# ohinder/OnePhase.jl

Hardware: AMD Instinct MI355X
Metric: KKT factor+solve/sec (fp64) at n+m~1e5, nnz~2e6 (higher is better)
Workload: dtype f64

## Files before the change

include/okkt.h:

```cpp
#ifndef OKKT_H
#define OKKT_H

#include <stdint.h>

#ifdef __cplusplus
extern "C" {
#endif

typedef struct okkt_solver_s* okkt_handle;
typedef struct okkt_kkt_s* okkt_kkt_handle;

typedef enum {
  OKKT_OK = 0,
  OKKT_ERR_INVALID = -1,
  OKKT_ERR_NO_DEVICE = -2,
  OKKT_ERR_HIP = -3,
  OKKT_ERR_ALLOC = -4,
  OKKT_ERR_INTERNAL = -5
} okkt_status;

#define OKKT_SYM_DEFINITE 0
#define OKKT_SYM_SYMMETRIC 1

#define OKKT_KKT_SCHUR 0
// ... 122 lines not shown
int okkt_get_schur_dev(okkt_handle h, double* d_S, int64_t ld);
int okkt_schur_condense(okkt_handle h, const double* rhs, double* r2, int64_t nrhs);
int okkt_schur_condense_dev(okkt_handle h, const double* d_rhs, double* d_r2, int64_t nrhs);
int okkt_schur_expand(okkt_handle h, const double* rhs, const double* x2, double* x, int64_t nrhs);
int okkt_schur_expand_dev(okkt_handle h, const double* d_rhs, const double* d_x2, double* d_x, int64_t nrhs);
int okkt_schur_factor(okkt_handle h, const double* S_or_NULL, int64_t ld, okkt_inertia* inertia_S, okkt_inertia* inertia_total);
int okkt_schur_factor_dev(okkt_handle h, const double* d_S_or_NULL, int64_t ld, okkt_inertia* inertia_S, okkt_inertia* inertia_total);
int okkt_schur_dense_solve(okkt_handle h, const double* r2, double* x2, int64_t nrhs);
int okkt_schur_dense_solve_dev(okkt_handle h, const double* d_r2, double* d_x2, int64_t nrhs);
int okkt_schur_solve(okkt_handle h, const double* rhs, double* sol, int64_t nrhs);
int okkt_schur_solve_dev(okkt_handle h, const double* d_rhs, double* d_sol, int64_t nrhs);
int okkt_schur_get_factor(okkt_handle h, double* LD, int64_t ld, int32_t* ipiv);
typedef struct {
  double seconds_device;
  int64_t arena_bytes;
  int64_t nonfinite;
  int32_t status;
  double flops;
} okkt_selinv_info;
int okkt_selinv(okkt_handle h, okkt_selinv_info* info );
int okkt_get_inverse_diag(okkt_handle h, double* d_out);
int okkt_get_inverse_diag_dev(okkt_handle h, double* d_out);
int okkt_get_inverse_on_pattern(okkt_handle h, double* zval, int64_t* nnz);
int okkt_get_inverse_on_pattern_dev(okkt_handle h, double* d_zval);
int okkt_get_inverse_csc(okkt_handle h, int64_t* colptr, int64_t* rowval, double* val, int64_t* nnz);
int okkt_logdet(okkt_handle h, double* logabsdet, int32_t* sign);

#define OKKT_SCALE_NONE 0
#define OKKT_SCALE_RUIZ 1
#define OKKT_SCALE_USER 2
typedef struct {
  int32_t mode, sweeps;
  double rowmax_min, rowmax_max;
  int64_t zero_rows;
} okkt_scaling_info;
int okkt_set_scaling(okkt_handle h, int mode, int32_t sweeps ,
                     const double* s_user );
int okkt_get_scaling(okkt_handle h, double* s_out , okkt_scaling_info* info );
int okkt_get_scaling_dev(okkt_handle h, double* d_s_out);

int okkt_get_diag(okkt_handle h, double* d_out );
int okkt_get_factor_csc(okkt_handle h, int64_t* colptr_out, int64_t* rowval_out, double* val_out, int64_t* nnz_out);

int okkt_dev_alloc(okkt_handle h, int64_t bytes, void** d_ptr_out);
int okkt_dev_free(okkt_handle h, void* d_ptr);
int okkt_dev_upload(okkt_handle h, void* d_dst, const void* src, int64_t bytes);
int okkt_dev_download(okkt_handle h, void* dst, const void* d_src, int64_t bytes);
int okkt_set_early_exit(okkt_handle h, int enable);
void* okkt_get_stream(okkt_handle h);
int okkt_profile_dominant(okkt_handle h, int enable);
int okkt_get_profile(okkt_handle h, int64_t* n_launches, double* total_ms, double* total_flops);
int64_t okkt_debug_dataflow_queue(int32_t nfronts, const int32_t* f, const int32_t* k, int32_t workers, int32_t group,
                                  int32_t* tasks, int64_t cap, double* model_us);


int okkt_dist_set_partition(okkt_handle h, int nparts, int part_id);
int okkt_dist_info(okkt_handle h, int64_t* cb_doubles, int64_t* cv_doubles, int64_t* n_boundary,
                   double* part_flops_out , double* top_flops_out);
int okkt_dist_get_owner(okkt_handle h, int64_t* sn_owner_out, int64_t* col_owner_out, int64_t* sn_parent_out);
int okkt_dist_factor_local(okkt_handle h, const double* d_nzval, int64_t n, int64_t m, int sym_kind);
int okkt_dist_cb(okkt_handle h, double* d_buf, int unpack);
int okkt_dist_factor_top(okkt_handle h);
int okkt_dist_counts(okkt_handle h, int64_t out[4]);
int okkt_dist_finish(okkt_handle h, const int64_t total[4]);
int okkt_dist_solve_begin(okkt_handle h, const double* d_rhs);
int okkt_dist_cv(okkt_handle h, double* d_buf, int unpack);
int okkt_dist_solve_top(okkt_handle h);
int okkt_dist_x(okkt_handle h, double* d_buf, int mode);
int okkt_dist_solve_end(okkt_handle h);

int okkt_dist_unique_id(void* id_out );
int okkt_dist_comm_init(okkt_handle h, int nranks, int rank, const void* id );
int okkt_dist_comm_destroy(okkt_handle h);
int okkt_dist_factor(okkt_handle h, const double* d_nzval, int64_t n, int64_t m, int sym_kind, okkt_inertia* inertia_out);
int okkt_dist_solve(okkt_handle h, const double* d_rhs, double* d_sol);

typedef struct {
  double delta_start, delta_min, delta_max, delta_inc, delta_dec, delta_zero;
  int32_t ItRefine_Num;
  int32_t max_it;
} okkt_kkt_pars;

typedef struct {
  double assemble_ms;
  double upload_ms;
  double shift_ms;
  double factor_ms;
  double rhs_ms;
  double solve_ms;
  double refine_ms;
  double kkt_err_ms;
  double direction_ms;
  int32_t n_solves;
  int32_t reserved;
} okkt_kkt_timers;

typedef struct {
  double error_D, error_P, error_mu, overall, rhs_norm, ratio;
} okkt_kkt_error;

int okkt_kkt_default_pars(okkt_kkt_pars* pars);
int okkt_kkt_create(okkt_kkt_handle* out, const okkt_opts* opts, int kkt_kind);
int okkt_kkt_destroy(okkt_kkt_handle k);
const char* okkt_kkt_last_error(okkt_kkt_handle k);
okkt_handle okkt_kkt_linear_solver(okkt_kkt_handle k);
int okkt_kkt_set_structure(okkt_kkt_handle k, int64_t n, int64_t m,
// ... 55 lines not shown
```

onephase.jl_amd/_lib.py:

```python
import ctypes as C
import os

import numpy as np

_HERE = os.path.dirname(os.path.abspath(__file__))
LIB_PATH = os.environ.get("OKKT_LIB_PATH", os.path.join(_HERE, "libonephase_kkt.so"))

OKKT_SYM_DEFINITE = 0
OKKT_SYM_SYMMETRIC = 1
OKKT_KKT_SCHUR = 0
OKKT_KKT_SYMMETRIC = 1
OKKT_KKT_CLEVER_SYMMETRIC = 2
OKKT_KKT_SCHUR_DIRECT = 3
OKKT_RESCALE = {"none": 0, "u_only": 1, "u_and_x": 2}
OKKT_SCALE_NONE = 0
OKKT_SCALE_RUIZ = 1
OKKT_SCALE_USER = 2
OKKT_SCALE = {"none": OKKT_SCALE_NONE, "ruiz": OKKT_SCALE_RUIZ, "user": OKKT_SCALE_USER}

OKKT_OK = 0
OKKT_ERR_INVALID = -1
OKKT_ERR_NO_DEVICE = -2
OKKT_ERR_HIP = -3
OKKT_ERR_ALLOC = -4
# ... 187 lines not shown
    "okkt_get_etree": (C.c_int, [_vp, _i64p, _i64p]),
    "okkt_factor": (C.c_int, [_vp, _f64p, C.c_int64, C.c_int64, C.c_int, C.POINTER(OkktInertia)]),
    "okkt_factor_dev": (C.c_int, [_vp, _vp, C.c_int64, C.c_int64, C.c_int, C.POINTER(OkktInertia)]),
    "okkt_solve": (C.c_int, [_vp, _f64p, _f64p, C.c_int64]),
    "okkt_solve_dev": (C.c_int, [_vp, _vp, _vp, C.c_int64]),
    "okkt_residual": (C.c_int, [_vp, _f64p, _f64p, _f64p, _f64p, C.c_int64, _f64p]),
    "okkt_residual_dev": (C.c_int, [_vp, _vp, _vp, _vp, _vp, C.c_int64, _f64p]),
    "okkt_solve_refine": (C.c_int, [_vp, _f64p, _f64p, _f64p, C.c_int64, C.c_int32, C.c_double, C.POINTER(OkktRefineInfo), _f64p]),
    "okkt_solve_refine_dev": (C.c_int, [_vp, _vp, _vp, _vp, C.c_int64, C.c_int32, C.c_double, C.POINTER(OkktRefineInfo), _f64p]),
    "okkt_solve_gmres": (C.c_int, [_vp, _f64p, _f64p, _f64p, C.c_int64, C.c_int32, C.c_int32, C.c_double, C.POINTER(OkktGmresInfo),
                                   _f64p]),
    "okkt_solve_gmres_dev": (C.c_int, [_vp, _vp, _vp, _vp, C.c_int64, C.c_int32, C.c_int32, C.c_double, C.POINTER(OkktGmresInfo), _f64p]),
    "okkt_condest": (C.c_int, [_vp, _f64p, C.c_int32, C.POINTER(OkktCondestInfo)]),
    "okkt_condest_dev": (C.c_int, [_vp, _vp, C.c_int32, C.POINTER(OkktCondestInfo)]),
    "okkt_condest_indices": (C.c_int64, [_vp, _i64p, C.c_int64]),
    "okkt_forward_error": (C.c_int, [_vp, _f64p, _f64p, _f64p, C.c_int64, _f64p, _f64p]),
    "okkt_forward_error_dev": (C.c_int, [_vp, _vp, _vp, _vp, C.c_int64, _f64p, _f64p]),
    "okkt_set_schur": (C.c_int, [_vp, C.c_int64, _i64p]),
    "okkt_factor_schur": (C.c_int, [_vp, _f64p, C.c_int64, C.c_int64, C.c_int, C.POINTER(OkktInertia)]),
    "okkt_factor_schur_dev": (C.c_int, [_vp, _vp, C.c_int64, C.c_int64, C.c_int, C.POINTER(OkktInertia)]),
    "okkt_get_schur": (C.c_int, [_vp, _f64p, C.c_int64]),
    "okkt_get_schur_dev": (C.c_int, [_vp, _vp, C.c_int64]),
    "okkt_schur_condense": (C.c_int, [_vp, _f64p, _f64p, C.c_int64]),
    "okkt_schur_condense_dev": (C.c_int, [_vp, _vp, _vp, C.c_int64]),
    "okkt_schur_expand": (C.c_int, [_vp, _f64p, _f64p, _f64p, C.c_int64]),
    "okkt_schur_expand_dev": (C.c_int, [_vp, _vp, _vp, _vp, C.c_int64]),
    "okkt_schur_factor": (C.c_int, [_vp, _f64p, C.c_int64, C.POINTER(OkktInertia), C.POINTER(OkktInertia)]),
    "okkt_schur_factor_dev": (C.c_int, [_vp, _vp, C.c_int64, C.POINTER(OkktInertia), C.POINTER(OkktInertia)]),
    "okkt_schur_dense_solve": (C.c_int, [_vp, _f64p, _f64p, C.c_int64]),
    "okkt_schur_dense_solve_dev": (C.c_int, [_vp, _vp, _vp, C.c_int64]),
    "okkt_schur_solve": (C.c_int, [_vp, _f64p, _f64p, C.c_int64]),
    "okkt_schur_solve_dev": (C.c_int, [_vp, _vp, _vp, C.c_int64]),
    "okkt_schur_get_factor": (C.c_int, [_vp, _f64p, C.c_int64, C.POINTER(C.c_int32)]),
    "okkt_selinv": (C.c_int, [_vp, C.POINTER(OkktSelinvInfo)]),
    "okkt_get_inverse_diag": (C.c_int, [_vp, _f64p]),
    "okkt_get_inverse_diag_dev": (C.c_int, [_vp, _vp]),
    "okkt_get_inverse_on_pattern": (C.c_int, [_vp, _f64p, _i64p]),
    "okkt_get_inverse_on_pattern_dev": (C.c_int, [_vp, _vp]),
    "okkt_get_inverse_csc": (C.c_int, [_vp, _i64p, _i64p, _f64p, _i64p]),
    "okkt_logdet": (C.c_int, [_vp, _f64p, C.POINTER(C.c_int32)]),
    "okkt_set_scaling": (C.c_int, [_vp, C.c_int, C.c_int32, _f64p]),
    "okkt_get_scaling": (C.c_int, [_vp, _f64p, C.POINTER(OkktScalingInfo)]),
    "okkt_get_scaling_dev": (C.c_int, [_vp, _vp]),
    "okkt_get_diag": (C.c_int, [_vp, _f64p]),
    "okkt_get_factor_csc": (C.c_int, [_vp, _i64p, _i64p, _f64p, _i64p]),
    "okkt_dev_alloc": (C.c_int, [_vp, C.c_int64, C.POINTER(_vp)]),
    "okkt_dev_free": (C.c_int, [_vp, _vp]),
    "okkt_dev_upload": (C.c_int, [_vp, _vp, _vp, C.c_int64]),
    "okkt_dev_download": (C.c_int, [_vp, _vp, _vp, C.c_int64]),
    "okkt_get_stream": (_vp, [_vp]),
    "okkt_profile_dominant": (C.c_int, [_vp, C.c_int]),
    "okkt_get_profile": (C.c_int, [_vp, _i64p, _f64p, _f64p]),
    "okkt_debug_dataflow_queue": (C.c_int64, [C.c_int32, C.POINTER(C.c_int32), C.POINTER(C.c_int32), C.c_int32, C.c_int32, C.POINTER(C.c_int32), C.c_int64, _f64p]),
    "okkt_dist_set_partition": (C.c_int, [_vp, C.c_int, C.c_int]),
    "okkt_dist_info": (C.c_int, [_vp, _i64p, _i64p, _i64p, _f64p, _f64p]),
    "okkt_dist_get_owner": (C.c_int, [_vp, _i64p, _i64p, _i64p]),
    "okkt_dist_factor_local": (C.c_int, [_vp, _vp, C.c_int64, C.c_int64, C.c_int]),
    "okkt_dist_cb": (C.c_int, [_vp, _vp, C.c_int]),
    "okkt_dist_factor_top": (C.c_int, [_vp]),
    "okkt_dist_counts": (C.c_int, [_vp, _i64p]),
    "okkt_dist_finish": (C.c_int, [_vp, _i64p]),
    "okkt_dist_solve_begin": (C.c_int, [_vp, _vp]),
    "okkt_dist_cv": (C.c_int, [_vp, _vp, C.c_int]),
    "okkt_dist_solve_top": (C.c_int, [_vp]),
    "okkt_dist_x": (C.c_int, [_vp, _vp, C.c_int]),
    "okkt_dist_solve_end": (C.c_int, [_vp]),
    "okkt_dist_unique_id": (C.c_int, [_vp]),
    "okkt_dist_comm_init": (C.c_int, [_vp, C.c_int, C.c_int, _vp]),
    "okkt_dist_comm_destroy": (C.c_int, [_vp]),
    "okkt_dist_factor": (C.c_int, [_vp, _vp, C.c_int64, C.c_int64, C.c_int, C.POINTER(OkktInertia)]),
    "okkt_dist_solve": (C.c_int, [_vp, _vp, _vp]),
    "okkt_kkt_default_pars": (C.c_int, [C.POINTER(OkktKktPars)]),
    "okkt_kkt_create": (C.c_int, [C.POINTER(_vp), C.POINTER(OkktOpts), C.c_int]),
    "okkt_kkt_destroy": (C.c_int, [_vp]),
    "okkt_kkt_last_error": (C.c_char_p, [_vp]),
    "okkt_kkt_linear_solver": (_vp, [_vp]),
    "okkt_kkt_set_structure": (C.c_int, [_vp, C.c_int64, C.c_int64, _i64p, _i64p, _i64p, _i64p, C.c_int]),
    "okkt_kkt_form_system": (C.c_int, [_vp, _f64p, _f64p, _f64p, _f64p]),
    "okkt_kkt_diag_min": (C.c_int, [_vp, _f64p]),
    "okkt_kkt_factor": (C.c_int, [_vp, C.c_double, C.POINTER(OkktInertia)]),
    "okkt_kkt_factor_trial": (C.c_int, [_vp, C.c_double, C.POINTER(OkktInertia)]),
    "okkt_kkt_get_timers": (C.c_int, [_vp, C.POINTER(OkktKktTimers)]),
    "okkt_kkt_get_direction": (C.c_int, [_vp, _f64p, _f64p, _f64p]),
    "okkt_kkt_ipopt_strategy": (C.c_int, [_vp, C.c_double, C.POINTER(OkktKktPars), C.POINTER(C.c_int32), _f64p]),
    "okkt_kkt_compute_directions": (C.c_int, [_vp, C.c_int32, _f64p, C.c_int32, _f64p, _f64p, _f64p, C.POINTER(OkktKktError)]),
    "okkt_kkt_is_diag_dom": (C.c_int, [_vp, C.POINTER(C.c_int32)]),
    "okkt_kkt_diag_dom_warnings": (C.c_int, [_vp, C.POINTER(C.c_int32)]),
    "okkt_kkt_estimate_y_tilde": (C.c_int, [_vp, _f64p, _f64p]),
    "okkt_kkt_system_rhs": (C.c_int, [_vp, _f64p, _f64p, _f64p, _f64p, _f64p, C.c_double, C.c_double, C.c_double, C.c_double, C.c_double, _f64p, _f64p, _f64p]),
    "okkt_kkt_compute_direction": (C.c_int, [_vp, _f64p, _f64p, _f64p, C.c_int32, _f64p, _f64p, _f64p, C.POINTER(OkktKktError)]),
    "okkt_kkt_get_matrix": (C.c_int, [_vp, _i64p, _i64p, _i64p, _i64p, _f64p]),
    "okkt_kkt_get_schur_diag": (C.c_int, [_vp, _f64p]),
    "okkt_kkt_get_dense_rows": (C.c_int, [_vp, _i64p, _i64p]),
    "okkt_kkt_set_ls_refine": (C.c_int, [_vp, C.c_int32, C.c_double]),
    "okkt_kkt_set_ls_scaling": (C.c_int, [_vp, C.c_int, C.c_int32]),
    "okkt_kkt_condest": (C.c_int, [_vp, C.c_int32, C.POINTER(OkktCondestInfo)]),
    "okkt_kkt_direction_error_bound": (C.c_int, [_vp, _f64p]),
    "okkt_kkt_compute_indicies": (C.c_int, [_vp, _f64p, C.POINTER(C.c_int64)]),
    "okkt_kkt_get_indicies": (C.c_int, [_vp, _i64p, _i64p, _i64p, _f64p, _f64p, _f64p, _f64p]),
    "okkt_kkt_get_clever_vectors": (C.c_int, [_vp, _f64p, _f64p, _f64p, _f64p, _f64p]),
    "okkt_kkt_set_rescale": (C.c_int, [_vp, C.c_int, C.c_double, C.c_double]),
    "okkt_kkt_set_direction": (C.c_int, [_vp, _f64p, _f64p, _f64p]),
    "okkt_kkt_max_step_primal": (C.c_int, [_vp, _f64p, C.c_double, _f64p, _f64p]),
    "okkt_kkt_s_bound_ok": (C.c_int, [_vp, _f64p, _f64p, C.c_double, C.POINTER(C.c_int32)]),
    "okkt_kkt_dual_step_range": (C.c_int, [_vp, _f64p, _f64p, C.c_double, C.c_double, _f64p, _f64p, _f64p]),
    "okkt_kkt_predicted_reduction": (C.c_int, [_vp, _f64p, C.c_double, C.c_double, C.c_double, C.c_double, _f64p]),
# ... 44 lines not shown
```

onephase.jl_amd/csrc/dataflow.hip:

```cpp
#include "front_device.h"

#include <algorithm>
#include <type_traits>
#include <cstdio>
#include <cstdlib>

namespace okkt {

#define OKKT_HIP_TRY(expr)                                                         \
  do {                                                                             \
    hipError_t e__ = (expr);                                                       \
    if (e__ != hipSuccess)                                                         \
      return std::string(#expr) + ": " + hipGetErrorString(e__);                   \
  } while (0)

typedef double d2_t __attribute__((ext_vector_type(2)));
constexpr int kDfThreadsC = 512;
#ifndef OKKT_DF_STAGES
#define OKKT_DF_STAGES 2
#endif
#ifndef OKKT_DF_KC
#define OKKT_DF_KC 32
#endif
#ifndef OKKT_DF_STAGGER
#define OKKT_DF_STAGGER 1
#endif
constexpr bool kDfStagger = OKKT_DF_STAGGER != 0;
#ifndef OKKT_DF_PROG
#define OKKT_DF_PROG 0
#endif
constexpr bool kDfProg = OKKT_DF_PROG != 0;
#ifndef OKKT_DF_MACRO
#define OKKT_DF_MACRO 0
#endif
#ifndef OKKT_DF_ROT
#define OKKT_DF_ROT 0
#endif
#ifndef OKKT_DF_CHAIN_BUILD
#define OKKT_DF_CHAIN_BUILD 0
#endif
constexpr bool kDfChain = OKKT_DF_CHAIN_BUILD != 0;
#ifndef OKKT_DF_LOG_BUILD
#define OKKT_DF_LOG_BUILD 0
#endif
constexpr bool kDfLog = OKKT_DF_LOG_BUILD != 0;
#ifndef OKKT_DF_PIPE
#define OKKT_DF_PIPE 0
#endif
#ifndef OKKT_DF_MULTI
#define OKKT_DF_MULTI 1
#endif
constexpr bool kDfMulti = OKKT_DF_MULTI != 0;
constexpr bool kDfPipe = OKKT_DF_PIPE != 0;
constexpr bool kDfRot = OKKT_DF_ROT != 0;
constexpr bool kDfMacro = OKKT_DF_MACRO != 0;
constexpr int kDfDiagMfmaWaves = 6;
constexpr int kDfKC = OKKT_DF_KC;
constexpr int kDfStages = OKKT_DF_STAGES;

__device__ __forceinline__ void st_sc1_f64x2(double* p, d2_t v) { asm volatile("global_store_dwordx4 %0, %1, off sc1" : : "v"(p), "v"(v) : "memory"); }
__device__ __forceinline__ int ld_state(const int* p) { return __hip_atomic_load(p, __ATOMIC_RELAXED, __HIP_MEMORY_SCOPE_AGENT); }

__device__ __forceinline__ int df_block_lo(int b, int KB, int k, int f) { return b < KB ? b * 128 : min(k + (b - KB) * 128, f); }

__device__ __forceinline__ void df_trsm_tile(const DevPlan& P, int s, int q, int r0, int rlim, double* sm) {
  constexpr int NBLK = 4, NB = 128, NPAIR = NBLK * (NBLK + 1) / 2;
  int tid_ = threadIdx.x;
  asm volatile("" : "+v"(tid_));
  const int tid = tid_, lane = tid & 63, wv = tid >> 6;
  const int col0 = P.sn_col0[s];
  const int k = P.sn_col0[s + 1] - col0;
  const int f = (int)(P.row_ptr[s + 1] - P.row_ptr[s]);
  const int j0 = q * NB;
  const int nb = min(NB, k - j0);
  double* F = P.arena + P.front_pos[s];
  double* Wb = P.wbuf + P.wbuf_pos[s] + (size_t)j0 * f;
  const double* X = P.invl + P.invl_pos[s] + (size_t)q * NB * NB;
  double* rdv = sm + NPAIR * kIB * kIB;
  const int row = r0 + wv * 16 + (lane & 15);
  const int rowc = min(row, f - 1);
  const bool valid = row < rlim;
  const int lk = lane >> 4, li = lane & 3;
  double t[NBLK * 8];
#pragma unroll
  for (int qq = 0; qq < NBLK * 8; ++qq) {
    const int c = 4 * qq + lk;
    t[qq] = keep_f64(F[(size_t)(j0 + min(c, nb - 1)) * f + rowc], c < nb && valid);
  }
  {
    const int e = tid * 2;
    const int cc = e / kIB, rr = e - cc * kIB;
#pragma unroll
    for (int bi = 0; bi < NBLK; ++bi)
#pragma unroll
      for (int bp = 0; bp <= bi; ++bp) {
        double v[2];
        const int gr = bi * kIB + rr, gc = bp * kIB + cc;
#pragma unroll
        for (int u = 0; u < 2; ++u) {
          const double* src = bp == bi ? X + (gr + u) + (size_t)gc * NB
                                       : F + (size_t)(j0 + min(gc, nb - 1)) * f + j0 + min(gr + u, nb - 1);
          v[u] = keep_f64(*src, gr + u < nb && gc < nb);
        }
        double* dst = sm + (bi * (bi + 1) / 2 + bp) * kIB * kIB + e;
        dst[0] = v[0]; dst[1] = v[1];
      }
    if (tid < NB) rdv[tid] = tid < nb ? 1.0 / P.dvals[col0 + j0 + tid] : 0.0;
// ... 712 lines not shown
#pragma unroll
      for (int cg = 0; cg < 4; ++cg) {
        const int c = r0 + 16 * (ucode[u] >> 2) + cg * 4 + l4;
        if (c >= rlim) continue;
        double* colp = F + (size_t)c * f;
        if (r + 1 < rlim && r >= c) {
          st_sc1_f64x2(colp + r, (d2_t){acc[u][cg][0], acc[u][cg][1]});
        } else {
          if (r < rlim && r >= c) st_agent_f64(colp + r, acc[u][cg][0]);
          if (r + 1 < rlim && r + 1 >= c) st_agent_f64(colp + r + 1, acc[u][cg][1]);
        }
      }
    }
    asm volatile("s_waitcnt vmcnt(0)" ::: "memory");
    __syncthreads();
    if (wave == 0) __hip_atomic_store(diag_state, dval, __ATOMIC_RELAXED, __HIP_MEMORY_SCOPE_AGENT);
  } else {
    asm volatile("s_waitcnt lgkmcnt(0)" ::: "memory");
    __syncthreads();
    double* Tl = sm;
#pragma unroll
    for (int u = 0; u < NU; ++u) {
      if (!unit_on(u)) continue;
      const int r = 32 * (ucode[u] & 3) + 2 * l15;
#pragma unroll
      for (int cg = 0; cg < 4; ++cg) {
        const int c = 16 * (ucode[u] >> 2) + cg * 4 + l4;
        const d2_t v = (d2_t){acc[u][cg][0], acc[u][cg][1]};
        __builtin_memcpy(Tl + (size_t)c * kDfTileLd + r, &v, 16);
      }
    }
    asm volatile("s_waitcnt vmcnt(0)" ::: "memory");
    __syncthreads();
    if (wave == 0) __hip_atomic_store(row_state, dval, __ATOMIC_RELAXED, __HIP_MEMORY_SCOPE_AGENT);
  }
  return true;
}

template <int CTRL>
__device__ __forceinline__ double df_row_ror(double v) {
  const int lo = __builtin_amdgcn_update_dpp(0, __double2loint(v), CTRL, 0xf, 0xf, false);
  const int hi = __builtin_amdgcn_update_dpp(0, __double2hiint(v), CTRL, 0xf, 0xf, false);
  return __hiloint2double(hi, lo);
}

template <int KC, int STAGES, bool MULTI, bool STAGGER>
__device__ __forceinline__ void df_syrk_tiles(const DevPlan& P, int s, int j0, int nb, int i, int R_, int j, int KB, int k, double* sm, long long* marks, int* pub0 = nullptr, int pub_stride = 0, int pub_val = 0) {
  constexpr int NW = kSyrkNW;
  constexpr int kDfKC = KC;
  const int R = MULTI ? R_ : 1;
  constexpr int DMA = 2 * (kDfKC / NW);
  constexpr int WCW = 128 / (NW / 2);
  constexpr int NCG = WCW / 4;
  int tid_ = threadIdx.x;
  asm volatile("" : "+v"(tid_));
  const int tid = tid_, lane = tid & 63, wv = tid >> 6;
  const int f = (int)(P.row_ptr[s + 1] - P.row_ptr[s]);
  const int ct0 = df_block_lo(j, KB, k, f), clim = df_block_lo(j + 1, KB, k, f);
  const int cbase = ct0 + (wv >> 1) * WCW;
  double* F = P.arena + P.front_pos[s];
  double* Fc = F + (j >= KB ? P.cb_shift[s] : 0);
  const double* Wcol = P.wbuf + P.wbuf_pos[s] + (size_t)j0 * f + lane * 2;
  const double* Lg = F + (size_t)j0 * f + ct0 + lane * 2;
  const int l15 = lane & 15, l4 = lane >> 4;
  const int quad = (lane >> 2) & 3;
  int grp1 = quad, grp2 = quad, grp3 = quad;
  if constexpr (kDfRot) {
    grp1 = __builtin_amdgcn_update_dpp(0, quad, 0x124, 0xf, 0xf, false);
    grp2 = __builtin_amdgcn_update_dpp(0, quad, 0x128, 0xf, 0xf, false);
    grp3 = __builtin_amdgcn_update_dpp(0, quad, 0x12C, 0xf, 0xf, false);
  }
  auto col_of = [&](int cg) {
    if constexpr (!kDfRot) return cbase + cg * 4 + l4;
    const int m = cg & 3;
    return cbase + (cg >> 2) * 16 + (m == 0 ? quad : m == 1 ? grp1 : m == 2 ? grp2 : grp3) * 4 + l4;
  };
  const int nchunk = (nb + kDfKC - 1) / kDfKC;
  const int total = R * nchunk;
  auto issue = [&](int g) {
    const int r = g / nchunk, ch = g - r * nchunk;
    const double* Wg = Wcol + df_block_lo(i + r, KB, k, f);
    double* slot = sm + (size_t)(g % STAGES) * 2 * kDfKC * kSyrkLd;
#pragma unroll
    for (int qq = 0; qq < kDfKC / NW; ++qq) {
      const int prow = qq * NW + wv;
      const int p = ch * kDfKC + prow;
      const double* wsrc = p < nb ? Wg + (size_t)p * f : P.zero_page + lane * 2;
      const double* lsrc = p < nb ? Lg + (size_t)p * f : P.zero_page + lane * 2;
      __builtin_amdgcn_global_load_lds(wsrc, (lds_void_t*)(slot + prow * kSyrkLd), 16, 0, 0);
      __builtin_amdgcn_global_load_lds(lsrc, (lds_void_t*)(slot + (kDfKC + prow) * kSyrkLd), 16, 0, 0);
    }
  };
  d2_t raw[NCG][2];
  auto load_c = [&](int r) {
    const int rbase = df_block_lo(i + r, KB, k, f) + (wv & 1) * 64;
#pragma unroll
    for (int cg = 0; cg < NCG; ++cg) {
      const int c = col_of(cg);
      const double* colp = Fc + (size_t)min(c, clim - 1) * f;
#pragma unroll
      for (int h = 0; h < 2; ++h) {
        const int rr = rbase + 2 * l15 + 32 * h;
        __builtin_memcpy(&raw[cg][h], colp + min(rr, f - 2), 16);
      }
    }
  };
  double acc[NCG][4];
  auto mask_c = [&](int r) {
    const int rbase = df_block_lo(i + r, KB, k, f) + (wv & 1) * 64;
    const int rlim = df_block_lo(i + r + 1, KB, k, f);
#pragma unroll
    for (int cg = 0; cg < NCG; ++cg) {
      const int c = col_of(cg);
#pragma unroll
      for (int h = 0; h < 2; ++h) {
        const int rr = rbase + 2 * l15 + 32 * h;
        const int shift = rr - min(rr, f - 2);
        const double e0 = shift == 0 ? raw[cg][h][0] : raw[cg][h][1];
        acc[cg][2 * h] = keep_f64(e0, rr < rlim && c < clim && rr >= c);
        acc[cg][2 * h + 1] = keep_f64(raw[cg][h][1], shift == 0 && rr + 1 < rlim && c < clim && rr + 1 >= c);
      }
    }
  };
  load_c(0);
  asm volatile("" ::: "memory");
  mask_c(0);
#pragma unroll
  for (int g = 0; g < STAGES - 1; ++g) if (g < total) issue(g);
  int pend_r = -1;
  int plain_until = 0;
  const int pre = min(2, nchunk - 1);
  int r = 0, ch = 0;
  for (int g = 0; g < total; ++g) {
    {
      const int later = g < plain_until ? 0 : min(STAGES - 2, total - 1 - g);
      if (later >= 2) asm volatile("s_waitcnt vmcnt(%0)" ::"n"(2 * DMA) : "memory");
      else if (later == 1) asm volatile("s_waitcnt vmcnt(%0)" ::"n"(DMA) : "memory");
      else asm volatile("s_waitcnt vmcnt(0)" ::: "memory");
    }
    __builtin_amdgcn_s_barrier();
    if constexpr (MULTI) {
      if (pend_r >= 0) {
        if (tid == 0) __hip_atomic_store(pub0 + (size_t)pend_r * pub_stride, pub_val, __ATOMIC_RELAXED, __HIP_MEMORY_SCOPE_AGENT);
        pend_r = -1;
      }
    }
    if (marks && g == 0 && tid == 0) { marks[0] = wall_clock64(); marks[3] = -(long long)clock64(); }
    const bool late = STAGGER && wv >= 4;
    const bool more = g + STAGES - 1 < total;
    if (more && !late) issue(g + STAGES - 1);
    if constexpr (MULTI) { if (ch == pre && r + 1 < R) { load_c(r + 1); plain_until = g + STAGES; } }
    const int rt0 = df_block_lo(i + r, KB, k, f), rlim = df_block_lo(i + r + 1, KB, k, f);
    const int rbase = rt0 + (wv & 1) * 64;
    const bool active = !(rbase + 63 < cbase) && rbase < rlim && cbase < clim && !(kDfChain && P.df_dbg_half && nb >= 256 && (g & 1));
    if (active) {
      const double* slot = sm + (size_t)(g % STAGES) * 2 * kDfKC * kSyrkLd;
      const double* bw = slot + (wv & 1) * 64 + 2 * l15;
      const double* bl = slot + kDfKC * kSyrkLd + (wv >> 1) * WCW + (kDfRot ? l15 : (lane & 3));
      if constexpr (kDfRot || !kDfPipe) {
  #pragma unroll
        for (int kk = 0; kk < kDfKC / 4; ++kk) {
          if (kk == (KC / 8) && more && late) issue(g + STAGES - 1);
          double bv[4];
  #pragma unroll
          for (int rb = 0; rb < 4; ++rb) bv[rb] = bw[(kk * 4 + l4) * kSyrkLd + (rb & 1) + 32 * (rb >> 1)];
  #pragma unroll
          for (int half = 0; half < NCG / 4; ++half) {
            double av[4];
  #pragma unroll
            for (int qq = 0; qq < 4; ++qq) if (!kDfRot || qq == 0) av[qq] = bl[(kk * 4 + l4) * kSyrkLd + (half * 4 + qq) * 4];
            if constexpr (kDfRot) {
              av[1] = df_row_ror<0x124>(av[0]);
              av[2] = df_row_ror<0x128>(av[0]);
              av[3] = df_row_ror<0x12C>(av[0]);
            }
  #pragma unroll
            for (int qq = 0; qq < 4; ++qq)
  #pragma unroll
              for (int rb = 0; rb < 4; ++rb)
                acc[half * 4 + qq][rb] = __builtin_amdgcn_mfma_f64_4x4x4f64(av[qq], bv[rb], acc[half * 4 + qq][rb], 0, 0, 1 );
          }
        }
      } else {
        static_assert(NCG == 8, "two halves of four column groups per k-step");
        const unsigned ba = (unsigned)(size_t)(bl + l4 * kSyrkLd);
        const unsigned bb = (unsigned)(size_t)(bw + l4 * kSyrkLd);
        d2_t B0[2], B1[2], A0[2], A1[2];
        auto ldb = [&](int kk, d2_t (&bq)[2]) {
          const unsigned ad = bb + kk * 4 * kSyrkLd * 8;
          asm volatile("ds_read_b128 %0, %2\n\tds_read_b128 %1, %2 offset:256" : "=&v"(bq[0]), "=&v"(bq[1]) : "v"(ad));
        };
        auto lda = [&](int kk, int half, d2_t (&aq)[2]) {
          const unsigned ad = ba + kk * 4 * kSyrkLd * 8 + half * 128;
          asm volatile("ds_read2_b64 %0, %2 offset1:4\n\tds_read2_b64 %1, %2 offset0:8 offset1:12" : "=&v"(aq[0]), "=&v"(aq[1]) : "v"(ad));
        };
        ldb(0, B0);
        lda(0, 0, A0);
#pragma unroll
        for (int st = 0; st < 2 * (kDfKC / 4); ++st) {
          const int kk = st >> 1, half = st & 1;
          d2_t (&Ac)[2] = (st & 1) ? A1 : A0;
          d2_t (&Bc)[2] = (kk & 1) ? B1 : B0;
          if (st == 2 * (KC / 8) && more && late) issue(g + STAGES - 1);
          if (st + 1 < 2 * (kDfKC / 4)) {
            const int k2 = (st + 1) >> 1, h2 = (st + 1) & 1;
            if (h2 == 0) ldb(k2, (k2 & 1) ? B1 : B0);
            lda(k2, h2, ((st + 1) & 1) ? A1 : A0);
          }
          if (st + 1 >= 2 * (kDfKC / 4)) asm volatile("s_waitcnt lgkmcnt(0)" : "+v"(Ac[0]), "+v"(Ac[1]), "+v"(Bc[0]), "+v"(Bc[1]));
          else if (((st + 1) & 1) == 0) asm volatile("s_waitcnt lgkmcnt(4)" : "+v"(Ac[0]), "+v"(Ac[1]), "+v"(Bc[0]), "+v"(Bc[1]));
          else asm volatile("s_waitcnt lgkmcnt(2)" : "+v"(Ac[0]), "+v"(Ac[1]), "+v"(Bc[0]), "+v"(Bc[1]));
#pragma unroll
          for (int qq = 0; qq < 4; ++qq)
#pragma unroll
            for (int rb = 0; rb < 4; ++rb)
              acc[half * 4 + qq][rb] = __builtin_amdgcn_mfma_f64_4x4x4f64(Ac[qq >> 1][qq & 1], Bc[rb >> 1][rb & 1], acc[half * 4 + qq][rb], 0, 0, 1 );
          __builtin_amdgcn_sched_barrier(0);
        }
      }
    } else if (more && late) issue(g + STAGES - 1);
    if (++ch == nchunk) {
      if (marks && g == total - 1 && tid == 0) { marks[1] = wall_clock64(); marks[3] += (long long)clock64(); }
      if (active) {
#pragma unroll
        for (int cg = 0; cg < NCG; ++cg) {
          const int c = col_of(cg);
          if (c >= clim) continue;
          double* colp = Fc + (size_t)c * f;
#pragma unroll
          for (int h = 0; h < 2; ++h) {
            const int rr = rbase + 2 * l15 + 32 * h;
            if (rr + 1 < rlim && rr >= c) {
              st_sc1_f64x2(colp + rr, (d2_t){acc[cg][2 * h], acc[cg][2 * h + 1]});
            } else {
              if (rr < rlim && rr >= c) st_agent_f64(colp + rr, acc[cg][2 * h]);
              if (rr + 1 < rlim && rr + 1 >= c) st_agent_f64(colp + rr + 1, acc[cg][2 * h + 1]);
            }
          }
        }
      }
      ch = 0;
      plain_until = g + STAGES;
      if constexpr (MULTI) { if (pub0 && r + 1 < R) pend_r = r; }
      ++r;
      if constexpr (MULTI) { if (r < R) mask_c(r); }
    }
  }
  if (marks && tid == 0) marks[2] = wall_clock64();
}

constexpr int kMacroKC = 16;
constexpr size_t kDfMacroLds = (size_t)2 * 3 * kMacroKC * kSyrkLd * sizeof(double);
__device__ __forceinline__ void df_syrk_macro(const DevPlan& P, int s, int j0, int nb, int i, int j, int KB, int k, double* sm, long long* marks) {
  constexpr int KC = kMacroKC, STAGES = 2;
  constexpr int DMA = 3 * KC / 8;
  int tid_ = threadIdx.x;
  asm volatile("" : "+v"(tid_));
  const int tid = tid_, lane = tid & 63, wv = tid >> 6;
  const int f = (int)(P.row_ptr[s + 1] - P.row_ptr[s]);
  const int ct0 = df_block_lo(j, KB, k, f), clim = df_block_lo(j + 1, KB, k, f);
  const int rt = wv & 1;
  const int cbase = ct0 + (wv >> 1) * 32;
  const int rt0 = df_block_lo(i + rt, KB, k, f), rlim = df_block_lo(i + rt + 1, KB, k, f);
  double* F = P.arena + P.front_pos[s];
  double* Fc = F + (j >= KB ? P.cb_shift[s] : 0);
  const double* Wcol = P.wbuf + P.wbuf_pos[s] + (size_t)j0 * f + lane * 2;
  const double* Lg = F + (size_t)j0 * f + ct0 + lane * 2;
  const int l15 = lane & 15, l4 = lane >> 4;
  const int nchunk = (nb + KC - 1) / KC;
  const int r0a = df_block_lo(i, KB, k, f), r0b = df_block_lo(i + 1, KB, k, f);
  static_assert(KC == 16, "the request pattern below deals 48 rows to eight waves: rows wv and 8 + wv of each of the three arrays");
  const double* wa = Wcol + r0a;
  const double* wb = Wcol + r0b;
  const double* zp = P.zero_page + lane * 2;
  auto issue = [&](int g) {
    double* slot = sm + (size_t)(g % STAGES) * 3 * KC * kSyrkLd;
#pragma unroll
    for (int qq = 0; qq < DMA; ++qq) {
      const int prow = (qq & 1) * 8 + wv;
// ... 253 lines not shown
          __builtin_amdgcn_fence(__ATOMIC_ACQUIRE, "agent");
          if (tlog && lane == 0) tlog[(size_t)qh * 8 + 1] = wall_clock64();
        }
        s_nxt[1] = qh; s_nxt[2] = rs; s_nxt[3] = rtn; s_nxt[4] = rij; s_nxt[5] = rq0;
        s_nxt[0] = ready ? 2 : 1;
        stage = 5;
      }
    }
    if (wave != 0 && looks && stage < 5) stage = stage + 1;
    {
      const int rbase = cur.rt0 + (wv & 1) * 64, cbase = cur.ct0 + (wv >> 1) * WCW;
      const bool active = !(rbase + 63 < cbase) && rbase < cur.rlim && cbase < cur.clim;
      if (active) {
        const double* slot = sm + (size_t)(G & 1) * 2 * KC * kSyrkLd;
        const double* bw = slot + (wv & 1) * 64 + 2 * l15;
        const double* bl = slot + KC * kSyrkLd + (wv >> 1) * WCW + (lane & 3);
#pragma unroll
        for (int kk = 0; kk < KC / 4; ++kk) {
          if (kk == (KC / 8) && more && late) issue_next();
          double bv[4];
#pragma unroll
          for (int rb = 0; rb < 4; ++rb) bv[rb] = bw[(kk * 4 + l4) * kSyrkLd + (rb & 1) + 32 * (rb >> 1)];
#pragma unroll
          for (int half = 0; half < NCG / 4; ++half) {
            double av[4];
#pragma unroll
            for (int qq = 0; qq < 4; ++qq) av[qq] = bl[(kk * 4 + l4) * kSyrkLd + (half * 4 + qq) * 4];
#pragma unroll
            for (int qq = 0; qq < 4; ++qq)
#pragma unroll
              for (int rb = 0; rb < 4; ++rb)
                acc[half * 4 + qq][rb] = __builtin_amdgcn_mfma_f64_4x4x4f64(av[qq], bv[rb], acc[half * 4 + qq][rb], 0, 0, 1 );
          }
        }
      } else if (more && late) issue_next();
    }
    ++G;
    if (!last) { ++c; continue; }
    store_c(cur);
    if (have != 2) break;
    pend = P.df_state + P.df_state_pos[cur.s] + (size_t)cur.i * cur.TB + cur.j; pendv = cur.q0 + cur.nq; pendt = cur.t;
    mask_c(nxt);
    cur = nxt;
    have = 0; c = 0; stage = 0;
    if (wave == 0) s_nxt[0] = 0;
  }
  *mine = P.df_state + P.df_state_pos[cur.s] + (size_t)cur.i * cur.TB + cur.j;
  *newv = cur.q0 + cur.nq;
  *t_last = cur.t;
  *t_claim = claimed;
}

constexpr int kDfThreads = kDfThreadsC;
constexpr size_t kDfLds = std::max(std::max(std::max(std::max(OKKT_DIAG2_LDS_DOUBLES(kMW) * sizeof(double), kDfTuLds), (size_t)kDfStages * 2 * kDfKC * kSyrkLd * sizeof(double)), kDfTlLds), std::max(std::max(kDfTuLockLds, kDfMacroLds), (size_t)128 * kDfTileLd * sizeof(double)));

__global__ __launch_bounds__(kDfThreads, 1) void k_front_dataflow(DevPlan P, const DfTask* __restrict__ tasks, int ntasks, int* __restrict__ head, double tol, int drop, int dbg, long long* __restrict__ tlog) {
  extern __shared__ __attribute__((aligned(16))) double sm[];
  __shared__ int s_ctl[8];
  __shared__ int s_nxt[8];
  const int tid = threadIdx.x;
  if constexpr (!kDfLog) { tlog = nullptr; dbg = 0; }
  const int wave = __builtin_amdgcn_readfirstlane(tid >> 6);
  int t_ahead = -1;
  for (;;) {
    if (wave == 0) {
      int t = t_ahead;
      if (t_ahead < 0) {
        if ((tid & 63) == 0) t = atomicAdd(head, 1);
        t = __builtin_amdgcn_readfirstlane(t);
      }
      int ok = 1;
      if (P.want_neg >= 0 && __builtin_amdgcn_readfirstlane((int)__hip_atomic_load(&P.counters[4], __ATOMIC_RELAXED, __HIP_MEMORY_SCOPE_AGENT)) != 0) ok = 0;
      if (tlog && t < ntasks && (tid & 63) == 0) { tlog[(size_t)t * 8] = wall_clock64(); tlog[(size_t)t * 8 + 3] = blockIdx.x; }
      if (t < ntasks && ok) {
        const DfTask tk = tasks[t];
        const int s = __builtin_amdgcn_readfirstlane(tk.front), type_nq = __builtin_amdgcn_readfirstlane(tk.type_nq), ij = __builtin_amdgcn_readfirstlane(tk.ij), q0 = __builtin_amdgcn_readfirstlane(tk.q0);
        const int type = type_nq & 255, nq = (type_nq >> 8) & 255, rows = max(type_nq >> 16, 1), i = ij & 0xffff, j = ij >> 16;
        const int k = P.sn_col0[s + 1] - P.sn_col0[s];
        const int f = (int)(P.row_ptr[s + 1] - P.row_ptr[s]);
        const int KB = (k + 127) >> 7;
        const int TB = KB + ((f - k + 127) >> 7);
        const int* st = P.df_state + P.df_state_pos[s];
        const int ln = tid & 63;
        const int* addr = st;
        int need = -(1 << 30);
        if (type == kDfD) { if (ln == 0) { addr = st + (size_t)i * TB + i; need = i; } }
        else if (type == kDfT) {
          if (ln == 0) { addr = st + (size_t)j * TB + j; need = j + 1; }
          if (ln == 1) { addr = st + (size_t)i * TB + j; need = j; }
        } else if (type == kDfTL) {
          if (ln == 0) { addr = st + (size_t)i * TB + j; need = j - 1; }
          if (ln == 1) { addr = st + (size_t)i * TB + (j - 1); need = j; }
          if (ln == 2) { addr = st + (size_t)j * TB + (j - 1); need = j; }
        } else if (type == kDfTU || type == kDfTA) {
          if (ln == 0) { addr = st + (size_t)i * TB + j; need = j; }
          if (ln == 1) { addr = st + (size_t)i * TB + i; need = j; }
        } else {
          const int ql = q0 + nq - 1;
          if (ln < rows) { addr = st + (size_t)(i + ln) * TB + ql; need = ql + 1; }
          else if (ln < 2 * rows) { addr = st + (size_t)(i + ln - rows) * TB + j; need = q0; }
          else if (ln == 2 * rows) { addr = st + (size_t)j * TB + ql; need = ql + 1; }
        }
        if (drop && ln == 0) need += 1 << 20;
        int spins = 0;
        long long t0w = 0;
        for (;;) {
          if (__builtin_amdgcn_ballot_w64(ld_state(addr) >= need) == ~0ull) break;
// ... 159 lines not shown
  if (!(e = up(all.data(), all.size() * sizeof(DfTask), (void**)&N.df_tasks)).empty()) return e;
  if (total + (int64_t)nheads * kDfHeadStride >= (int64_t)1 << 31) return "dataflow: tile states beyond 2^31";
  {
    void* p = nullptr;
    const size_t bytes = ((size_t)total + (size_t)nheads * kDfHeadStride + 16) * sizeof(int);
    OKKT_HIP_TRY(hipMalloc(&p, bytes));
    N.allocations.push_back(p);
    OKKT_HIP_TRY(hipMemset(p, 0, bytes));
    OKKT_HIP_TRY(hipStreamSynchronize(nullptr));
    d.df_state = (int*)p;
    N.df_heads = d.df_state + total;
  }
  return "";
}

std::string df_launch(Numeric& N, const DevPlan& P, const Segment& g, hipStream_t st, double tol) {
  if (g.df_cnt <= 0) return "";
  static const int drop = getenv("OKKT_DEBUG_DROP_HANDOFF") ? atoi(getenv("OKKT_DEBUG_DROP_HANDOFF")) : 0;
  static const int dbg_env = getenv("OKKT_DEBUG_DATAFLOW") ? atoi(getenv("OKKT_DEBUG_DATAFLOW")) : 0;
  static const int dbg = kDfLog ? dbg_env : (dbg_env & 8);
  static const bool warned = [] {
    if (!kDfLog && (dbg_env & ~8)) fprintf(stderr, "okkt: OKKT_DEBUG_DATAFLOW=%d: the task log and the body switches are compiled into libonephase_kkt_log.so and libonephase_kkt_exp.so only (OKKT_LIB_PATH); ignored here\n", dbg_env);
    return true;
  }();
  (void)warned;
  const int grid = std::min(g.df_cnt, N.df_workers);
  long long* tlog = nullptr;
  if (dbg & 16) { OKKT_HIP_TRY(hipMalloc((void**)&tlog, (size_t)g.df_cnt * 8 * sizeof(long long))); OKKT_HIP_TRY(hipMemsetAsync(tlog, 0, (size_t)g.df_cnt * 8 * sizeof(long long), st)); }
  hipLaunchKernelGGL(k_front_dataflow, dim3(grid), dim3(kDfThreads), kDfLds, st, P, N.df_tasks + g.df_off, g.df_cnt, N.df_heads + g.df_head * kDfHeadStride, tol, (drop & 4) ? 1 : 0, dbg, tlog);
  if (dbg & 24) {
    hipError_t e2 = hipStreamSynchronize(st);
    fprintf(stderr, "okkt: dataflow launch of %d tasks on %d workers: %s\n", g.df_cnt, grid, hipGetErrorString(e2));
  }
  if (tlog) {
    std::vector<long long> hl((size_t)g.df_cnt * 8);
    std::vector<DfTask> ht((size_t)g.df_cnt);
    OKKT_HIP_TRY(hipMemcpy(hl.data(), tlog, hl.size() * sizeof(long long), hipMemcpyDeviceToHost));
    OKKT_HIP_TRY(hipMemcpy(ht.data(), N.df_tasks + g.df_off, ht.size() * sizeof(DfTask), hipMemcpyDeviceToHost));
    (void)hipFree(tlog);
    const char* path = getenv("OKKT_DF_LOG");
    if (FILE* fp = fopen(path ? path : "/tmp/okkt_df_log.txt", "a")) {
      fprintf(fp, "# launch %d tasks %d workers (index front type i j q0 nq worker pop ready end [10 ns ticks])\n", g.df_cnt, grid);
      for (int t = 0; t < g.df_cnt; ++t)
        fprintf(fp, "%d %d %d %d %d %d %d %lld %lld %lld %lld %lld %lld %lld %lld\n", t, ht[t].front, ht[t].type_nq & 255, ht[t].ij & 0xffff, ht[t].ij >> 16, ht[t].q0, ht[t].type_nq >> 8,
                hl[(size_t)t * 8 + 3], hl[(size_t)t * 8], hl[(size_t)t * 8 + 1], hl[(size_t)t * 8 + 2], hl[(size_t)t * 8 + 4], hl[(size_t)t * 8 + 5], hl[(size_t)t * 8 + 6], hl[(size_t)t * 8 + 7]);
      fclose(fp);
    }
  }
  OKKT_HIP_TRY(hipGetLastError());
  return "";
}

}
```

Measured before the change: 55.14.

## Use contiguous fragment column map and tighter LDS ring strides in dataflow SYRK

Adds a new fragment mapping (enabled by default) where each lane owns eight contiguous columns, so the A operand for four MFMAs comes from two 16-byte vector LDS loads. The LDS ring strides shrink from 144 to 128/130 doubles, which cuts ring LDS footprint and changes bank mapping. The epilogue store column mapping is updated to match, and a debug query function exposes the fragment maps. It risks bank conflicts under the new strides and leaves the rotation and pipelined variants incompatible with this map.

```diff
diff --git a/include/okkt.h b/include/okkt.h
--- a/include/okkt.h
+++ b/include/okkt.h
@@ -198,6 +198,7 @@
 int okkt_get_profile(okkt_handle h, int64_t* n_launches, double* total_ms, double* total_flops);
 int64_t okkt_debug_dataflow_queue(int32_t nfronts, const int32_t* f, const int32_t* k, int32_t workers, int32_t group,
                                   int32_t* tasks, int64_t cap, double* model_us);
+int64_t okkt_debug_dataflow_fragment(int32_t map, int32_t what, int32_t wave, int32_t lane, int32_t kk, int32_t idx);
 
 
 int okkt_dist_set_partition(okkt_handle h, int nparts, int part_id);
diff --git a/onephase.jl_amd/_lib.py b/onephase.jl_amd/_lib.py
--- a/onephase.jl_amd/_lib.py
+++ b/onephase.jl_amd/_lib.py
@@ -263,6 +263,7 @@
     "okkt_profile_dominant": (C.c_int, [_vp, C.c_int]),
     "okkt_get_profile": (C.c_int, [_vp, _i64p, _f64p, _f64p]),
     "okkt_debug_dataflow_queue": (C.c_int64, [C.c_int32, C.POINTER(C.c_int32), C.POINTER(C.c_int32), C.c_int32, C.c_int32, C.POINTER(C.c_int32), C.c_int64, _f64p]),
+    "okkt_debug_dataflow_fragment": (C.c_int64, [C.c_int32] * 6),
     "okkt_dist_set_partition": (C.c_int, [_vp, C.c_int, C.c_int]),
     "okkt_dist_info": (C.c_int, [_vp, _i64p, _i64p, _i64p, _f64p, _f64p]),
     "okkt_dist_get_owner": (C.c_int, [_vp, _i64p, _i64p, _i64p]),
diff --git a/onephase.jl_amd/csrc/dataflow.hip b/onephase.jl_amd/csrc/dataflow.hip
--- a/onephase.jl_amd/csrc/dataflow.hip
+++ b/onephase.jl_amd/csrc/dataflow.hip
@@ -1,4 +1,6 @@
 #include "front_device.h"
+#include "df_fragments.h"
+#include "../../include/okkt.h"
 
 #include <algorithm>
 #include <type_traits>
@@ -53,6 +55,13 @@
 constexpr bool kDfMulti = OKKT_DF_MULTI != 0;
 constexpr bool kDfPipe = OKKT_DF_PIPE != 0;
 constexpr bool kDfRot = OKKT_DF_ROT != 0;
+#ifndef OKKT_DF_CONTIG
+#define OKKT_DF_CONTIG 1
+#endif
+constexpr int kDfContig = OKKT_DF_CONTIG != 0 ? 1 : 0;
+static_assert(!(kDfContig && (OKKT_DF_ROT != 0 || OKKT_DF_PIPE != 0)), "the rotation and hand-pipelined experiments are written for the earlier fragment map");
+static_assert(kDfFragLdOld == kSyrkLd, "df_fragments.h describes the earlier ring with kSyrkLd");
+static_assert(df_ring_rot(kDfContig, 1) == 0, "the LDS-DMA of df_syrk_tiles fetches a panel column lane-linearly");
 constexpr bool kDfMacro = OKKT_DF_MACRO != 0;
 constexpr int kDfDiagMfmaWaves = 6;
 constexpr int kDfKC = OKKT_DF_KC;
@@ -871,6 +880,8 @@
   constexpr int DMA = 2 * (kDfKC / NW);
   constexpr int WCW = 128 / (NW / 2);
   constexpr int NCG = WCW / 4;
+  constexpr int LDW = df_ring_ld_w(kDfContig), LDL = df_ring_ld_l(kDfContig), SLOT = df_ring_slot_doubles(kDfContig, kDfKC);
+  static_assert(WCW == 32 && NCG == 8, "df_fragments.h: 2 x 4 waves of 64 rows x 32 columns");
   int tid_ = threadIdx.x;
   asm volatile("" : "+v"(tid_));
   const int tid = tid_, lane = tid & 63, wv = tid >> 6;
@@ -890,7 +901,7 @@
     grp3 = __builtin_amdgcn_update_dpp(0, quad, 0x12C, 0xf, 0xf, false);
   }
   auto col_of = [&](int cg) {
-    if constexpr (!kDfRot) return cbase + cg * 4 + l4;
+    if constexpr (!kDfRot) return cbase + df_frag_acc_col(kDfContig, lane, cg);
     const int m = cg & 3;
     return cbase + (cg >> 2) * 16 + (m == 0 ? quad : m == 1 ? grp1 : m == 2 ? grp2 : grp3) * 4 + l4;
   };
@@ -899,15 +910,15 @@
   auto issue = [&](int g) {
     const int r = g / nchunk, ch = g - r * nchunk;
     const double* Wg = Wcol + df_block_lo(i + r, KB, k, f);
-    double* slot = sm + (size_t)(g % STAGES) * 2 * kDfKC * kSyrkLd;
+    double* slot = sm + (size_t)(g % STAGES) * SLOT;
 #pragma unroll
     for (int qq = 0; qq < kDfKC / NW; ++qq) {
       const int prow = qq * NW + wv;
       const int p = ch * kDfKC + prow;
       const double* wsrc = p < nb ? Wg + (size_t)p * f : P.zero_page + lane * 2;
       const double* lsrc = p < nb ? Lg + (size_t)p * f : P.zero_page + lane * 2;
-      __builtin_amdgcn_global_load_lds(wsrc, (lds_void_t*)(slot + prow * kSyrkLd), 16, 0, 0);
-      __builtin_amdgcn_global_load_lds(lsrc, (lds_void_t*)(slot + (kDfKC + prow) * kSyrkLd), 16, 0, 0);
+      __builtin_amdgcn_global_load_lds(wsrc, (lds_void_t*)(slot + prow * LDW), 16, 0, 0);
+      __builtin_amdgcn_global_load_lds(lsrc, (lds_void_t*)(slot + kDfKC * LDW + prow * LDL), 16, 0, 0);
     }
   };
   d2_t raw[NCG][2];
@@ -973,10 +984,29 @@
     const int rbase = rt0 + (wv & 1) * 64;
     const bool active = !(rbase + 63 < cbase) && rbase < rlim && cbase < clim && !(kDfChain && P.df_dbg_half && nb >= 256 && (g & 1));
     if (active) {
-      const double* slot = sm + (size_t)(g % STAGES) * 2 * kDfKC * kSyrkLd;
+      const double* slot = sm + (size_t)(g % STAGES) * SLOT;
       const double* bw = slot + (wv & 1) * 64 + 2 * l15;
       const double* bl = slot + kDfKC * kSyrkLd + (wv >> 1) * WCW + (kDfRot ? l15 : (lane & 3));
-      if constexpr (kDfRot || !kDfPipe) {
+      if constexpr (kDfContig) {
+  #pragma unroll
+        for (int kk = 0; kk < kDfKC / 4; ++kk) {
+          if (kk == (KC / 8) && more && late) issue(g + STAGES - 1);
+          d2_t bq[2];
+  #pragma unroll
+          for (int h = 0; h < 2; ++h) bq[h] = *(const d2_t*)(slot + df_frag_b_off(kDfContig, wv, lane, kk, 2 * h));
+  #pragma unroll
+          for (int half = 0; half < NCG / 4; ++half) {
+            d2_t aq[2];
+  #pragma unroll
+            for (int h = 0; h < 2; ++h) aq[h] = *(const d2_t*)(slot + df_frag_a_off(kDfContig, kDfKC, wv, lane, kk, half * 4 + 2 * h));
+  #pragma unroll
+            for (int qq = 0; qq < 4; ++qq)
+  #pragma unroll
+              for (int rb = 0; rb < 4; ++rb)
+                acc[half * 4 + qq][rb] = __builtin_amdgcn_mfma_f64_4x4x4f64(aq[qq >> 1][qq & 1], bq[rb >> 1][rb & 1], acc[half * 4 + qq][rb], 0, 0, 1 );
+          }
+        }
+      } else if constexpr (kDfRot || !kDfPipe) {
   #pragma unroll
         for (int kk = 0; kk < kDfKC / 4; ++kk) {
           if (kk == (KC / 8) && more && late) issue(g + STAGES - 1);
@@ -1041,9 +1071,11 @@
     if (++ch == nchunk) {
       if (marks && g == total - 1 && tid == 0) { marks[1] = wall_clock64(); marks[3] += (long long)clock64(); }
       if (active) {
+        int lane_s = lane;
+        if constexpr (kDfContig) asm volatile("v_mbcnt_lo_u32_b32 %0, -1, 0\n\tv_mbcnt_hi_u32_b32 %0, -1, %0" : "=v"(lane_s));
 #pragma unroll
         for (int cg = 0; cg < NCG; ++cg) {
-          const int c = col_of(cg);
+          const int c = kDfContig ? cbase + df_frag_acc_col(kDfContig, lane_s, cg) : col_of(cg);
           if (c >= clim) continue;
           double* colp = Fc + (size_t)c * f;
 #pragma unroll
@@ -1403,7 +1435,7 @@
 }
 
 constexpr int kDfThreads = kDfThreadsC;
-constexpr size_t kDfLds = std::max(std::max(std::max(std::max(OKKT_DIAG2_LDS_DOUBLES(kMW) * sizeof(double), kDfTuLds), (size_t)kDfStages * 2 * kDfKC * kSyrkLd * sizeof(double)), kDfTlLds), std::max(std::max(kDfTuLockLds, kDfMacroLds), (size_t)128 * kDfTileLd * sizeof(double)));
+constexpr size_t kDfLds = std::max(std::max(std::max(std::max(OKKT_DIAG2_LDS_DOUBLES(kMW) * sizeof(double), kDfTuLds), (size_t)kDfStages * df_ring_slot_doubles(kDfContig, kDfKC) * sizeof(double)), kDfTlLds), std::max(std::max(kDfTuLockLds, kDfMacroLds), (size_t)128 * kDfTileLd * sizeof(double)));
 
 __global__ __launch_bounds__(kDfThreads, 1) void k_front_dataflow(DevPlan P, const DfTask* __restrict__ tasks, int ntasks, int* __restrict__ head, double tol, int drop, int dbg, long long* __restrict__ tlog) {
   extern __shared__ __attribute__((aligned(16))) double sm[];
@@ -1669,3 +1701,21 @@
 }
 
 }
+
+extern "C" int64_t okkt_debug_dataflow_fragment(int32_t map, int32_t what, int32_t wave, int32_t lane, int32_t kk, int32_t idx) {
+  using namespace okkt;
+  if (map < 0) map = kDfContig;
+  if (map > 1 || wave < 0 || wave >= 8 || lane < 0 || lane >= 64 || kk < 0 || kk >= kDfKC / 4 || idx < 0 || idx >= 8) return OKKT_ERR_INVALID;
+  switch (what) {
+    case 0: return df_frag_acc_col(map, lane, idx);
+    case 1: return df_frag_a_col(map, lane, idx);
+    case 2: return df_frag_a_off(map, kDfKC, wave, lane, kk, idx);
+    case 3: return idx < 4 ? df_frag_b_off(map, wave, lane, kk, idx) : OKKT_ERR_INVALID;
+    case 4: return df_ring_rot(map, 4 * kk + (lane >> 4));
+    case 5: {
+      const int64_t geo[8] = {df_ring_ld_w(map), df_ring_ld_l(map), df_ring_slot_doubles(map, kDfKC), kDfKC, kDfStages, kDfContig, (int64_t)kDfLds, kSyrkLd};
+      return geo[idx];
+    }
+  }
+  return OKKT_ERR_INVALID;
+}
diff --git a/onephase.jl_amd/csrc/df_fragments.h b/onephase.jl_amd/csrc/df_fragments.h
--- /dev/null
+++ b/onephase.jl_amd/csrc/df_fragments.h
@@ -0,0 +1,28 @@
+#pragma once
+
+#if defined(__HIPCC__)
+#define OKKT_FRAG_HD __host__ __device__
+#else
+#define OKKT_FRAG_HD
+#endif
+
+namespace okkt {
+
+constexpr int kDfFragLdOld = 144;
+
+OKKT_FRAG_HD constexpr int df_ring_ld_w(int map) { return map ? 128 : kDfFragLdOld; }
+OKKT_FRAG_HD constexpr int df_ring_ld_l(int map) { return map ? 130 : kDfFragLdOld; }
+OKKT_FRAG_HD constexpr int df_ring_slot_doubles(int map, int kc) { return kc * (df_ring_ld_w(map) + df_ring_ld_l(map)); }
+OKKT_FRAG_HD constexpr int df_ring_rot(int map, int p) { return 0 * (map + p); }
+
+OKKT_FRAG_HD constexpr int df_frag_acc_col(int map, int lane, int cg) { return map ? 8 * (lane >> 4) + cg : 4 * cg + (lane >> 4); }
+OKKT_FRAG_HD constexpr int df_frag_a_col(int map, int lane, int cg) { return map ? 8 * (lane & 3) + cg : 4 * cg + (lane & 3); }
+
+OKKT_FRAG_HD constexpr int df_frag_a_off(int map, int kc, int wave, int lane, int kk, int cg) {
+  return kc * df_ring_ld_w(map) + (4 * kk + (lane >> 4)) * df_ring_ld_l(map) + 32 * (wave >> 1) + df_frag_a_col(map, lane, cg);
+}
+OKKT_FRAG_HD constexpr int df_frag_b_off(int map, int wave, int lane, int kk, int rb) {
+  return (4 * kk + (lane >> 4)) * df_ring_ld_w(map) + 64 * (wave & 1) + 2 * (lane & 15) + (rb & 1) + 32 * (rb >> 1);
+}
+
+}
```

After: 55.88, median of 6. +1.3%, better.
